# NVIDIA-Merlin/NVTabular

Hardware: NVIDIA H100
Metric: rows/sec Criteo-1TB-shaped Categorify+FillMissing+Normalize (higher is better)
Workload: dtype int64

## Files before the change

### nvtabular_b200/csrc/bucketagg.cuh

```cuda
#pragma once

namespace nvtb {

constexpr int kBkThreads = 1024;
constexpr int kBkLgParts = 13;
constexpr int kBkParts = 1 << kBkLgParts;
constexpr int kBkMaxShift = 32 - kBkLgParts;
constexpr int kBkWords = 1 << (kBkMaxShift - 5);
constexpr int kBkDupCap = 14336;
constexpr int kBkCountSmem = 4 * kBkWords;
constexpr int kBkEmitSmem = 4 * kBkWords * 2 + 2 * kBkWords + 4 * kBkDupCap;

struct PartRange {
  int lg;
  const uint32_t* par;
  __device__ __forceinline__ uint32_t xform(uint32_t k) const { return (k ^ 0x80000000u) - par[0]; }
  __device__ __forceinline__ uint32_t bin(uint32_t v) const { return v >> par[1]; }
};

static __global__ void __launch_bounds__(kPartThreads)
bk_minmax_kernel(const int32_t* __restrict__ keys, const uint8_t* __restrict__ mask, int64_t n,
                 uint32_t* __restrict__ mm, int aligned) {
  uint32_t lo = 0xFFFFFFFFu, hi = 0u;
  const int64_t n_tiles = (n + kPartTile - 1) / kPartTile;
  for (int64_t tile = blockIdx.x; tile < n_tiles; tile += gridDim.x) {
    Rows8 r[kPartGroups];
#pragma unroll
    for (int g = 0; g < kPartGroups; ++g)
      load_rows8(keys, mask, tile * kPartTile + ((int64_t)g * kPartThreads + threadIdx.x) * 8, n, r[g], aligned != 0);
#pragma unroll
    for (int g = 0; g < kPartGroups; ++g)
#pragma unroll
      for (int k = 0; k < 8; ++k)
        if ((r[g].m >> k) & 1u) {
          const uint32_t u = (uint32_t)r[g].v[k] ^ 0x80000000u;
          lo = u < lo ? u : lo;
          hi = u > hi ? u : hi;
        }
  }
#pragma unroll
  for (int o = 16; o > 0; o >>= 1) {
    const uint32_t a = __shfl_down_sync(0xFFFFFFFFu, lo, o), b = __shfl_down_sync(0xFFFFFFFFu, hi, o);
    lo = a < lo ? a : lo;
    hi = b > hi ? b : hi;
  }
  if ((threadIdx.x & 31) == 0 && lo <= hi) { atomicMin(&mm[0], lo); atomicMax(&mm[1], hi); }
}

static __global__ void bk_params_kernel(const uint32_t* __restrict__ mm, uint32_t* __restrict__ par) {
  uint32_t lo = mm[0], hi = mm[1];
  if (lo > hi) { lo = 0u; hi = 0u; }
  const uint32_t range = hi - lo;
  const int bits = range ? 32 - __clz(range) : 0;
  par[0] = lo;
  par[1] = (uint32_t)(bits > kBkLgParts ? bits - kBkLgParts : 0);
}

__device__ __forceinline__ uint32_t bk_block_sum(uint32_t v, uint32_t* ws ) {
#pragma unroll
  for (int o = 16; o > 0; o >>= 1) v += __shfl_down_sync(0xFFFFFFFFu, v, o);
  if ((threadIdx.x & 31) == 0) ws[threadIdx.x >> 5] = v;
  __syncthreads();
  uint32_t t = 0;
  if (threadIdx.x < 32) {
    t = ws[threadIdx.x];
#pragma unroll
    for (int o = 16; o > 0; o >>= 1) t += __shfl_down_sync(0xFFFFFFFFu, t, o);
    if (threadIdx.x == 0) ws[0] = t;
  }
  __syncthreads();
  t = ws[0];
  __syncthreads();
  return t;
}

__device__ __forceinline__ uint32_t bk_block_excl(uint32_t v, uint32_t* ws , uint32_t* total) {
  uint32_t incl = v;
#pragma unroll
  for (int o = 1; o < 32; o <<= 1) {
    const uint32_t y = __shfl_up_sync(0xFFFFFFFFu, incl, o);
    if ((threadIdx.x & 31) >= o) incl += y;
  }
  if ((threadIdx.x & 31) == 31) ws[threadIdx.x >> 5] = incl;
  __syncthreads();
  if (threadIdx.x < 32) {
    const uint32_t w = ws[threadIdx.x];
    uint32_t wi = w;
#pragma unroll
    for (int o = 1; o < 32; o <<= 1) {
      const uint32_t y = __shfl_up_sync(0xFFFFFFFFu, wi, o);
      if (threadIdx.x >= o) wi += y;
    }
    ws[threadIdx.x] = wi - w;
    if (threadIdx.x == 31) ws[32] = wi;
  }
  __syncthreads();
  const uint32_t ex = ws[threadIdx.x >> 5] + incl - v;
  *total = ws[32];
  __syncthreads();
  return ex;
}

static __global__ void __launch_bounds__(kBkThreads)
bk_count_kernel(const uint32_t* __restrict__ buf, const uint32_t* __restrict__ starts,
                const uint32_t* __restrict__ n_valid, const uint32_t* __restrict__ par,
                uint32_t* __restrict__ distinct) {
  extern __shared__ __align__(16) uint32_t bk_smem[];
  __shared__ uint32_t ws[33];
  uint32_t* bm = bk_smem;
  const int b = blockIdx.x;
  const uint32_t s = starts[b], e = (b + 1 < kBkParts) ? starts[b + 1] : *n_valid;
  if (s >= e) { if (threadIdx.x == 0) distinct[b] = 0u; return; }
  const uint32_t shift = par[1];
  const uint32_t wmask = (1u << shift) - 1u;
  const int words = shift > 5 ? 1 << (shift - 5) : 1;
  for (int w = threadIdx.x; w < words; w += kBkThreads) bm[w] = 0u;
  __syncthreads();
  for (uint32_t i = s + threadIdx.x; i < e; i += kBkThreads) {
    const uint32_t off = buf[i] & wmask;
    const uint32_t bit = 1u << (off & 31);
    if (!(bm[off >> 5] & bit)) atomicOr(&bm[off >> 5], bit);
  }
  __syncthreads();
  uint32_t c = 0;
  for (int w = threadIdx.x; w < words; w += kBkThreads) c += __popc(bm[w]);
  const uint32_t tot = bk_block_sum(c, ws);
  if (threadIdx.x == 0) distinct[b] = tot;
}

static __global__ void __launch_bounds__(kBkThreads)
bk_emit_kernel(const uint32_t* __restrict__ buf, const uint32_t* __restrict__ starts,
               const uint32_t* __restrict__ n_valid, const uint32_t* __restrict__ par,
               const uint32_t* __restrict__ out_base, uint64_t* __restrict__ out,
               unsigned int* __restrict__ flag, unsigned long long* __restrict__ max_count) {
  extern __shared__ __align__(16) uint32_t bk_smem[];
  __shared__ uint32_t ws[33];
  uint32_t* bm = bk_smem;
  uint32_t* dup = bm + kBkWords;
  uint16_t* pfx = reinterpret_cast<uint16_t*>(dup + kBkWords);
  uint32_t* cnt = reinterpret_cast<uint32_t*>(pfx + kBkWords);
  const int b = blockIdx.x;
  const uint32_t s = starts[b], e = (b + 1 < kBkParts) ? starts[b + 1] : *n_valid;
  if (s >= e) return;
  const uint32_t lo = par[0], shift = par[1];
  const uint32_t wmask = (1u << shift) - 1u;
  const int words = shift > 5 ? 1 << (shift - 5) : 1;
  const int per = (words + kBkThreads - 1) / kBkThreads;
  for (int w = threadIdx.x; w < words; w += kBkThreads) { bm[w] = 0u; dup[w] = 0u; }
  __syncthreads();
  for (uint32_t i = s + threadIdx.x; i < e; i += kBkThreads) {
    const uint32_t off = buf[i] & wmask;
    const uint32_t bit = 1u << (off & 31), w = off >> 5;
    const uint32_t old = atomicOr(&bm[w], bit);
    if ((old & bit) && !(dup[w] & bit)) atomicOr(&dup[w], bit);
  }
  __syncthreads();
  const int w0 = threadIdx.x * per;
  uint32_t c = 0;
  for (int j = 0; j < per; ++j) if (w0 + j < words) c += __popc(dup[w0 + j]);
  uint32_t n_dup;
  uint32_t run = bk_block_excl(c, ws, &n_dup);
  if (n_dup > (uint32_t)kBkDupCap) {
    if (threadIdx.x == 0) atomicOr(flag, 1u);
    return;
  }
  for (int j = 0; j < per; ++j)
    if (w0 + j < words) { pfx[w0 + j] = (uint16_t)run; run += __popc(dup[w0 + j]); }
  for (uint32_t i = threadIdx.x; i < n_dup; i += kBkThreads) cnt[i] = 0u;
  __syncthreads();
  if (n_dup) {
    for (uint32_t i = s + threadIdx.x; i < e; i += kBkThreads) {
      const uint32_t off = buf[i] & wmask;
      const uint32_t bit = 1u << (off & 31), w = off >> 5;
      const uint32_t d = dup[w];
      if (d & bit) atomicAdd(&cnt[pfx[w] + __popc(d & (bit - 1u))], 1u);
    }
    __syncthreads();
  }
  c = 0;
  for (int j = 0; j < per; ++j) if (w0 + j < words) c += __popc(bm[w0 + j]);
  uint32_t n_out;
  uint32_t r = bk_block_excl(c, ws, &n_out);
  uint64_t* o = out + out_base[b];
  const uint32_t vbase = lo + ((uint32_t)b << shift);
  uint32_t mx = 1u;
  for (int j = 0; j < per; ++j) {
    const int w = w0 + j;
    if (w >= words) break;
    uint32_t bits = bm[w];
    const uint32_t d = dup[w];
    const uint32_t pd = pfx[w];
    while (bits) {
      const int k = __ffs(bits) - 1;
      bits &= bits - 1u;
      uint32_t n = 1u;
      if ((d >> k) & 1u) n = cnt[pd + __popc(d & ((1u << k) - 1u))];
      mx = n > mx ? n : mx;
      o[r++] = ((uint64_t)(vbase + ((uint32_t)w << 5) + (uint32_t)k) << 32) | (uint64_t)n;
    }
  }
#pragma unroll
  for (int o2 = 16; o2 > 0; o2 >>= 1) { const uint32_t y = __shfl_down_sync(0xFFFFFFFFu, mx, o2); mx = y > mx ? y : mx; }
  if ((threadIdx.x & 31) == 0) atomicMax(max_count, (unsigned long long)mx);
}

}
```

### nvtabular_b200/csrc/sortacc.cu

```cuda
#include <algorithm>
#include <new>

#include "hashagg.cuh"
#include "partition.cuh"
#include "sortagg.cuh"
#include "bucketagg.cuh"

namespace nvtb {

struct SortedAcc {
  uint64_t* acc[2] = {nullptr, nullptr};
  int64_t acc_cap[2] = {0, 0};
  int cur = 0;
  uint32_t* d_n = nullptr;
  int32_t* stage_keys = nullptr;
  uint8_t* stage_mask = nullptr;
  int64_t stage_cap = 0;
  int64_t stage_rows = 0;
  int64_t stage_hint = 0;
  cudaEvent_t stage_ev = nullptr;
  cudaStream_t stage_last = nullptr;
};

static SharedScratch g_sort;

struct SortCarve {
  void* rx;
  size_t rx_bytes;
  uint32_t* part_meta;
  uint32_t* keys_a;
  uint32_t* keys_b;
  uint64_t* rle;
  uint32_t* tile_heads;
  uint2* splits;
  uint32_t* tile_out;
};

static size_t align_up(size_t v, size_t a) { return (v + a - 1) / a * a; }

static int sort_scratch_acquire(int64_t m, int64_t n_pairs_sort, int64_t mt, cudaStream_t st, SortCarve* c) {
  const int P = 1 << kSortLowBits;
  const size_t rx_bytes = align_up(std::max(rx_scratch_bytes<uint32_t>(m), rx_scratch_bytes<uint64_t>(n_pairs_sort)), 256);
  const size_t meta_bytes = align_up(sizeof(uint32_t) * (size_t)std::max(3 * P, 4 * kBkParts + 64), 256);
  const size_t keys_bytes = align_up(sizeof(uint32_t) * (size_t)(m + 64), 256);
  const size_t rle_bytes = align_up(sizeof(uint64_t) * (size_t)(m + 2), 256);
  const size_t heads_bytes = align_up(sizeof(uint32_t) * (size_t)((m + kRleTile - 1) / kRleTile + 1), 256);
  const size_t splits_bytes = align_up(sizeof(uint2) * (size_t)(mt + 2), 256);
  const size_t out_bytes = align_up(sizeof(uint32_t) * (size_t)(mt + 2), 256);
  const size_t need = rx_bytes + meta_bytes + 2 * keys_bytes + rle_bytes + heads_bytes + splits_bytes + out_bytes;
  void* base = nullptr;
  bool grown = false;
  int rc = g_sort.acquire(need, need + need / 8, st, &base, &grown);
  if (rc) return rc;
  if (grown) NVTB_CUDA_OK(cudaMemsetAsync(base, 0, 256, st));
  char* p = reinterpret_cast<char*>(base);
  c->rx = p;                                         p += rx_bytes;
  c->rx_bytes = rx_bytes;
  c->part_meta = reinterpret_cast<uint32_t*>(p);     p += meta_bytes;
  c->keys_a = reinterpret_cast<uint32_t*>(p);        p += keys_bytes;
  c->keys_b = reinterpret_cast<uint32_t*>(p);        p += keys_bytes;
  c->rle = reinterpret_cast<uint64_t*>(p);           p += rle_bytes;
  c->tile_heads = reinterpret_cast<uint32_t*>(p);    p += heads_bytes;
  c->splits = reinterpret_cast<uint2*>(p);           p += splits_bytes;
  c->tile_out = reinterpret_cast<uint32_t*>(p);
  return NVTB_OK;
}

static int acc_reserve(SortedAcc* a, int which, int64_t pairs, cudaStream_t st) {
  if (a->acc_cap[which] >= pairs) return NVTB_OK;
  if (a->acc[which]) NVTB_CUDA_OK(cudaFreeAsync(a->acc[which], st));
  a->acc[which] = nullptr; a->acc_cap[which] = 0;
  const int64_t want = pairs + pairs / 8 + 1024;
  NVTB_CUDA_OK(cudaMallocAsync(&a->acc[which], sizeof(uint64_t) * (size_t)want, st));
  a->acc_cap[which] = want;
  return NVTB_OK;
}

template <bool B_PACKED>
static int merge_pairs(const uint64_t* A, int64_t ua, const uint64_t* B, const uint32_t* ub_dev, int64_t mt,
                       uint64_t* out, unsigned long long* n_unique, unsigned long long* max_count, uint2* splits,
                       uint32_t* tile_out, cudaStream_t st) {
  static bool attrs = false;
  if (!attrs) {
    NVTB_CUDA_OK(cudaFuncSetAttribute(merge_write_kernel<B_PACKED>,
                                      cudaFuncAttributeMaxDynamicSharedMemorySize, (int)sizeof(MergeSmem)));
    attrs = true;
  }
  merge_split_kernel<<<(int)((mt + 1 + 255) / 256), 256, 0, st>>>(A, (uint32_t)ua, B, ub_dev, (int)mt, splits);
  NVTB_LAUNCH_OK();
  merge_count_kernel<<<(int)mt, kRunThreads, 0, st>>>(A, B, splits, tile_out);
  NVTB_LAUNCH_OK();
  scan_tiles_kernel<<<1, kRunThreads, 0, st>>>(tile_out, (int)mt, nullptr, n_unique);
  NVTB_LAUNCH_OK();
  merge_write_kernel<B_PACKED><<<(int)mt, kRunThreads, sizeof(MergeSmem), st>>>(A, B, splits, tile_out, out, max_count);
  NVTB_LAUNCH_OK();
  return NVTB_OK;
}

static int bucket_route(SortedAcc* a, const int32_t* kp, const uint8_t* mp, int64_t m, int64_t ua, Counters* ctr,
                        const SortCarve& c, cudaStream_t st, bool* ok) {
  static bool attrs = false;
  constexpr int kBkScatterSmem = kPartTile * 4 + 2 * 4 * kBkParts;
  if (!attrs) {
    NVTB_CUDA_OK(cudaFuncSetAttribute(part_hist_kernel<PartRange>, cudaFuncAttributeMaxDynamicSharedMemorySize, 4 * kBkParts));
    NVTB_CUDA_OK(cudaFuncSetAttribute(part_scatter_kernel<PartRange>, cudaFuncAttributeMaxDynamicSharedMemorySize, kBkScatterSmem));
    NVTB_CUDA_OK(cudaFuncSetAttribute(bk_count_kernel, cudaFuncAttributeMaxDynamicSharedMemorySize, kBkCountSmem));
    NVTB_CUDA_OK(cudaFuncSetAttribute(bk_emit_kernel, cudaFuncAttributeMaxDynamicSharedMemorySize, kBkEmitSmem));
    attrs = true;
  }
  const int sms = sm_count();
  const int aligned = is_aligned32(kp) ? 1 : 0;
  const int64_t tiles = (m + kPartTile - 1) / kPartTile;
  uint32_t* n_valid = a->d_n + 1;
  uint32_t* n_batch = a->d_n + 2;
  uint32_t* total = c.part_meta;
  uint32_t* cursor = c.part_meta + kBkParts;
  uint32_t* distinct = c.part_meta + 2 * kBkParts;
  uint32_t* mm = c.part_meta + 4 * kBkParts;
  uint32_t* par = mm + 2;
  unsigned int* flag = reinterpret_cast<unsigned int*>(mm + 4);
  const uint32_t mm_init[6] = {0xFFFFFFFFu, 0u, 0u, 0u, 0u, 0u};
  NVTB_CUDA_OK(cudaMemcpyAsync(mm, mm_init, sizeof(mm_init), cudaMemcpyHostToDevice, st));
  NVTB_CUDA_OK(cudaMemsetAsync(total, 0, sizeof(uint32_t) * kBkParts, st));
  bk_minmax_kernel<<<(int)std::min<int64_t>(tiles, 4 * sms), kPartThreads, 0, st>>>(kp, mp, m, mm, aligned);
  NVTB_LAUNCH_OK();
  bk_params_kernel<<<1, 1, 0, st>>>(mm, par);
  NVTB_LAUNCH_OK();
  const PartRange pol{kBkLgParts, par};
  part_hist_kernel<PartRange><<<(int)std::min<int64_t>(tiles, 3 * sms), kPartThreads, 4 * kBkParts, st>>>(
      kp, mp, m, pol, total, ctr, aligned);
  NVTB_LAUNCH_OK();
  scan_tiles_kernel<<<1, kRunThreads, 0, st>>>(total, kBkParts, n_valid, nullptr);
  NVTB_LAUNCH_OK();
  NVTB_CUDA_OK(cudaMemcpyAsync(cursor, total, sizeof(uint32_t) * kBkParts, cudaMemcpyDeviceToDevice, st));
  part_scatter_kernel<PartRange><<<(int)std::min<int64_t>(tiles, sms), kPartThreads, kBkScatterSmem, st>>>(
      kp, mp, m, pol, cursor, reinterpret_cast<int32_t*>(c.keys_a), aligned);
  NVTB_LAUNCH_OK();
  bk_count_kernel<<<kBkParts, kBkThreads, kBkCountSmem, st>>>(c.keys_a, total, n_valid, par, distinct);
  NVTB_LAUNCH_OK();
  scan_tiles_kernel<<<1, kRunThreads, 0, st>>>(distinct, kBkParts, n_batch, ua == 0 ? &ctr->n_unique : nullptr);
  NVTB_LAUNCH_OK();
  uint32_t nb_h = 0;
  NVTB_CUDA_OK(cudaMemcpyAsync(&nb_h, n_batch, sizeof(nb_h), cudaMemcpyDeviceToHost, st));
  NVTB_CUDA_OK(cudaStreamSynchronize(st));
  int rc = acc_reserve(a, a->cur ^ 1, ua + (int64_t)nb_h, st);
  if (rc) return rc;
  uint64_t* B = (ua == 0) ? a->acc[a->cur ^ 1] : c.rle;
  bk_emit_kernel<<<kBkParts, kBkThreads, kBkEmitSmem, st>>>(c.keys_a, total, n_valid, par, distinct, B, flag,
                                                             &ctr->max_count);
  NVTB_LAUNCH_OK();
  unsigned int flag_h = 0;
  NVTB_CUDA_OK(cudaMemcpyAsync(&flag_h, flag, sizeof(flag_h), cudaMemcpyDeviceToHost, st));
  NVTB_CUDA_OK(cudaStreamSynchronize(st));
  *ok = (flag_h == 0);
  return NVTB_OK;
}

static int radix_route(SortedAcc* a, const int32_t* kp, const uint8_t* mp, int64_t m, int64_t ua, Counters* null_ctr,
                       const SortCarve& c, cudaStream_t st) {
  static bool attrs = false;
  constexpr int kScatterSmem = kPartTile * 4 + 2 * 4 * (1 << kSortLowBits);
  if (!attrs) {
    NVTB_CUDA_OK(cudaFuncSetAttribute(part_scatter_kernel<PartKeyLow>,
                                      cudaFuncAttributeMaxDynamicSharedMemorySize, kScatterSmem));
    attrs = true;
  }
  const int sms = sm_count();
  const int P = 1 << kSortLowBits;
  const int aligned = is_aligned32(kp) ? 1 : 0;
  const int64_t tiles = (m + kPartTile - 1) / kPartTile;
  uint32_t* n_valid = a->d_n + 1;
  uint32_t* n_batch = a->d_n + 2;
  int rc = acc_reserve(a, a->cur ^ 1, ua + m, st);
  if (rc) return rc;
  NVTB_CUDA_OK(cudaMemsetAsync(c.part_meta, 0, sizeof(uint32_t) * P, st));
  part_hist_kernel<PartKeyLow><<<(int)std::min<int64_t>(tiles, 3 * sms), kPartThreads, 4 * P, st>>>(
      kp, mp, m, PartKeyLow{kSortLowBits}, c.part_meta, null_ctr, aligned);
  NVTB_LAUNCH_OK();
  part_scan_kernel<<<1, kPartThreads, 0, st>>>(c.part_meta, kSortLowBits, c.part_meta + P, c.part_meta + 2 * P, 1u, n_valid);
  NVTB_LAUNCH_OK();
  part_scatter_kernel<PartKeyLow><<<(int)std::min<int64_t>(tiles, 2 * sms), kPartThreads, kScatterSmem, st>>>(
      kp, mp, m, PartKeyLow{kSortLowBits}, c.part_meta + 2 * P, reinterpret_cast<int32_t*>(c.keys_a), aligned);
  NVTB_LAUNCH_OK();
  int in_b = 0;
  rc = rx_sort_bits<uint32_t>(nullptr, c.keys_a, c.keys_b, n_valid, m, kSortLowBits, 32, false, c.rx, c.rx_bytes, st,
                              &in_b);
  if (rc) return rc;
  const uint32_t* sorted = in_b ? c.keys_b : c.keys_a;
  const int rt = (int)((m + kRleTile - 1) / kRleTile);
  rle_count_kernel<<<rt, kRunThreads, 0, st>>>(sorted, n_valid, m, c.tile_heads);
  NVTB_LAUNCH_OK();
  scan_tiles_kernel<<<1, kRunThreads, 0, st>>>(c.tile_heads, rt, n_batch, nullptr);
  NVTB_LAUNCH_OK();
  rle_write_kernel<<<rt, kRunThreads, 0, st>>>(sorted, n_valid, m, c.tile_heads, n_batch, c.rle);
  NVTB_LAUNCH_OK();
  return NVTB_OK;
}

int sortacc_insert(SortedAcc* a, const int32_t* kp, const uint8_t* mp, int64_t m, int64_t ua, Counters* ctr,
                   cudaStream_t st) {
  const int64_t mt = (ua + m + kMergeTile - 1) / kMergeTile;
  SortCarve c;
  int rc = sort_scratch_acquire(m, 64, mt, st, &c);
  if (rc) return rc;
  const char* path_env = getenv("NVTB_SORT_PATH");
  const bool radix_only = path_env && strcmp(path_env, "radix") == 0;
  bool bucketed = false;
  if (!radix_only) {
    rc = bucket_route(a, kp, mp, m, ua, ctr, c, st, &bucketed);
    if (rc) return rc;
  }
  if (!bucketed) {
    rc = radix_route(a, kp, mp, m, ua, radix_only ? ctr : nullptr, c, st);
    if (rc) return rc;
  }
  const uint64_t* A = a->acc[a->cur];
  uint64_t* out = a->acc[a->cur ^ 1];
  uint32_t* n_batch = a->d_n + 2;
  if (!bucketed)
    rc = merge_pairs<false>(A, ua, c.rle, n_batch, mt, out, &ctr->n_unique, &ctr->max_count, c.splits, c.tile_out, st);
  else if (ua > 0)
    rc = merge_pairs<true>(A, ua, c.rle, n_batch, mt, out, &ctr->n_unique, &ctr->max_count, c.splits, c.tile_out, st);
  if (rc) return rc;
  a->cur ^= 1;
  return g_sort.release(st);
}

static int64_t stage_cap_rows() {
  const char* e = getenv("NVTB_STAGE_ROWS");
  int64_t v = e ? atoll(e) : ((int64_t)1 << 28);
  if (v < 0) v = 0;
  if (v > (int64_t)0xF0000000ll) v = (int64_t)0xF0000000ll;
  return v / 64 * 64;
}

int sortacc_create(SortedAcc** out, int64_t u, cudaStream_t st, uint64_t** pairs) {
  SortedAcc* a = new (std::nothrow) SortedAcc();
  NVTB_REQUIRE(a != nullptr, "host allocation failed");
  *out = a;
  *pairs = nullptr;
  NVTB_CUDA_OK(cudaMalloc(&a->d_n, sizeof(uint32_t) * 4));
  NVTB_CUDA_OK(cudaMemsetAsync(a->d_n, 0, sizeof(uint32_t) * 4, st));
  if (u > 0) {
    int rc = acc_reserve(a, 0, u, st);
    if (rc) return rc;
    rc = acc_reserve(a, 1, u, st);
    if (rc) return rc;
    *pairs = a->acc[0];
  }
  return NVTB_OK;
}

int sortacc_sort_pairs(SortedAcc* a, int64_t u, cudaStream_t st) {
  if (u == 0) return NVTB_OK;
  SortCarve c;
  int rc = sort_scratch_acquire(64, u, 1, st, &c);
  if (rc) return rc;
  int in_b = 0;
  rc = rx_sort_bits<uint64_t>(nullptr, a->acc[0], a->acc[1], nullptr, u, 32, 64, false, c.rx, c.rx_bytes, st, &in_b);
  if (rc) return rc;
  a->cur = in_b;
  return g_sort.release(st);
}

bool sortacc_stages(const SortedAcc* a, int64_t m) {
  const int64_t cap = stage_cap_rows();
  return cap >= 64 && m <= cap && (a->stage_rows & 7) == 0;
}

bool sortacc_stage_full(const SortedAcc* a, int64_t m) {
  return a->stage_rows > 0 && a->stage_rows + m > a->stage_cap;
}

int64_t sortacc_staged_rows(const SortedAcc* a) { return a->stage_rows; }

int sortacc_stage(SortedAcc* a, const int32_t* kp, const uint8_t* mp, int64_t m, int64_t rows_total, cudaStream_t st) {
  if (a->stage_ev == nullptr) NVTB_CUDA_OK(cudaEventCreateWithFlags(&a->stage_ev, cudaEventDisableTiming));
  if (a->stage_last != nullptr && a->stage_last != st) NVTB_CUDA_OK(cudaStreamWaitEvent(st, a->stage_ev, 0));
  const int64_t cap_max = stage_cap_rows();
  const bool grow_for_fit = a->stage_rows == 0 && a->stage_cap < std::min<int64_t>(cap_max, a->stage_hint);
  if (a->stage_rows + m > a->stage_cap || grow_for_fit) {
    NVTB_REQUIRE(a->stage_rows == 0, "staging buffer resized while rows are waiting");
    if (a->stage_keys) NVTB_CUDA_OK(cudaFreeAsync(a->stage_keys, st));
    if (a->stage_mask) NVTB_CUDA_OK(cudaFreeAsync(a->stage_mask, st));
    a->stage_keys = nullptr; a->stage_mask = nullptr; a->stage_cap = 0;
    int64_t want = (int64_t)1 << 22;
    while (want < 2 * (rows_total + m)) want <<= 1;
    want = std::max<int64_t>(want, (a->stage_hint + 63) / 64 * 64);
    want = std::max<int64_t>(std::min<int64_t>(want, cap_max), m);
    NVTB_CUDA_OK(cudaMallocAsync(&a->stage_keys, sizeof(int32_t) * (size_t)(want + 64), st));
    NVTB_CUDA_OK(cudaMallocAsync(&a->stage_mask, (size_t)(want / 8 + 64), st));
    a->stage_cap = want;
  }
  NVTB_CUDA_OK(cudaMemcpyAsync(a->stage_keys + a->stage_rows, kp, sizeof(int32_t) * (size_t)m, cudaMemcpyDeviceToDevice, st));
  uint8_t* md = a->stage_mask + (a->stage_rows >> 3);
  const size_t mbytes = (size_t)((m + 7) >> 3);
  if (mp) NVTB_CUDA_OK(cudaMemcpyAsync(md, mp, mbytes, cudaMemcpyDeviceToDevice, st));
  else    NVTB_CUDA_OK(cudaMemsetAsync(md, 0xFF, mbytes, st));
  a->stage_rows += m;
  NVTB_CUDA_OK(cudaEventRecord(a->stage_ev, st));
  a->stage_last = st;
  return NVTB_OK;
}

int sortacc_flush(SortedAcc* a, int64_t u, Counters* ctr, cudaStream_t st) {
  if (a->stage_rows == 0) return NVTB_OK;
  if (a->stage_last != st && a->stage_ev) NVTB_CUDA_OK(cudaStreamWaitEvent(st, a->stage_ev, 0));
  int rc = sortacc_insert(a, a->stage_keys, a->stage_mask, a->stage_rows, u, ctr, st);
  if (rc) return rc;
  a->stage_rows = 0;
  NVTB_CUDA_OK(cudaEventRecord(a->stage_ev, st));
  a->stage_last = st;
  return NVTB_OK;
}

void sortacc_reset(SortedAcc* a, int64_t rows_total) {
  a->stage_hint = std::max<int64_t>(a->stage_hint, rows_total);
  a->stage_rows = 0;
}

void sortacc_destroy(SortedAcc* a) {
  if (a->acc[0]) cudaFree(a->acc[0]);
  if (a->acc[1]) cudaFree(a->acc[1]);
  if (a->d_n) cudaFree(a->d_n);
  if (a->stage_keys) cudaFree(a->stage_keys);
  if (a->stage_mask) cudaFree(a->stage_mask);
  if (a->stage_ev) cudaEventDestroy(a->stage_ev);
  delete a;
}

const uint64_t* sortacc_pairs(const SortedAcc* a) { return a->acc[a->cur]; }

int sortacc_unpack(const SortedAcc* a, int64_t u, int64_t* keys, int64_t* sizes, cudaStream_t st) {
  runs_unpack_kernel<<<plain_grid(u), kThreads, 0, st>>>(a->acc[a->cur], u, keys, sizes);
  NVTB_LAUNCH_OK();
  return NVTB_OK;
}

}

using namespace nvtb;

extern "C" {

static int radix_sort_entry(void* data, void* tmp, int64_t n, int elem_bytes, int lo_bit, int hi_bit,
                            int descending, int* result_in_tmp_host, void* stream) {
  NVTB_REQUIRE(n >= 0 && result_in_tmp_host != nullptr, "bad n / NULL result flag");
  NVTB_REQUIRE(lo_bit >= 0 && hi_bit <= 8 * elem_bytes && lo_bit <= hi_bit, "bad bit range");
  *result_in_tmp_host = 0;
  if (n == 0 || lo_bit == hi_bit) return NVTB_OK;
  NVTB_REQUIRE(data != nullptr && tmp != nullptr, "NULL data/tmp");
  NVTB_REQUIRE((reinterpret_cast<uintptr_t>(data) & 15u) == 0 && (reinterpret_cast<uintptr_t>(tmp) & 15u) == 0,
               "data/tmp must be 16-byte aligned");
  cudaStream_t st = (cudaStream_t)stream;
  void* scratch = nullptr;
  const size_t bytes = elem_bytes == 4 ? rx_scratch_bytes<uint32_t>(n) : rx_scratch_bytes<uint64_t>(n);
  NVTB_CUDA_OK(cudaMallocAsync(&scratch, bytes, st));
  NVTB_CUDA_OK(cudaMemsetAsync(scratch, 0, 256, st));
  int rc;
  if (elem_bytes == 4)
    rc = rx_sort_bits<uint32_t>(nullptr, (uint32_t*)data, (uint32_t*)tmp, nullptr, n, lo_bit, hi_bit, descending != 0,
                                scratch, bytes, st, result_in_tmp_host);
  else
    rc = rx_sort_bits<uint64_t>(nullptr, (uint64_t*)data, (uint64_t*)tmp, nullptr, n, lo_bit, hi_bit, descending != 0,
                                scratch, bytes, st, result_in_tmp_host);
  NVTB_CUDA_OK(cudaFreeAsync(scratch, st));
  return rc;
}

int nvtb_radix_sort_u32(uint32_t* data, uint32_t* tmp, int64_t n, int lo_bit, int hi_bit, int descending,
                        int* result_in_tmp_host, void* stream) {
  return radix_sort_entry(data, tmp, n, 4, lo_bit, hi_bit, descending, result_in_tmp_host, stream);
}

int nvtb_radix_sort_u64(uint64_t* data, uint64_t* tmp, int64_t n, int lo_bit, int hi_bit, int descending,
                        int* result_in_tmp_host, void* stream) {
  return radix_sort_entry(data, tmp, n, 8, lo_bit, hi_bit, descending, result_in_tmp_host, stream);
}

int nvtb_pairs_lower_bounds(const uint64_t* pairs, int64_t n, const uint32_t* bounds_dev, int m,
                            int64_t* out_dev, void* stream) {
  NVTB_REQUIRE(n >= 0 && m >= 0, "negative size");
  if (m == 0) return NVTB_OK;
  NVTB_REQUIRE(bounds_dev != nullptr && out_dev != nullptr && (n == 0 || pairs != nullptr), "NULL argument");
  pairs_lower_bound_kernel<<<(m + 127) / 128, 128, 0, (cudaStream_t)stream>>>(
      pairs, n, bounds_dev, m, reinterpret_cast<long long*>(out_dev));
  NVTB_LAUNCH_OK();
  return NVTB_OK;
}

int nvtb_pairs_merge(const uint64_t* a, int64_t na, const uint64_t* b, int64_t nb, uint64_t* out,
                     int64_t* n_out_host, void* stream) {
  NVTB_REQUIRE(na >= 0 && nb >= 0 && n_out_host != nullptr, "bad sizes / NULL n_out");
  NVTB_REQUIRE(na + nb < (int64_t)0xFFFF0000ll, "more than 2^32 pairs in one merge");
  cudaStream_t st = (cudaStream_t)stream;
  *n_out_host = 0;
  if (na + nb == 0) return NVTB_OK;
  NVTB_REQUIRE(out != nullptr, "NULL out");
  if (na == 0 || nb == 0) {
    NVTB_CUDA_OK(cudaMemcpyAsync(out, na ? a : b, sizeof(uint64_t) * (size_t)(na + nb), cudaMemcpyDeviceToDevice, st));
    *n_out_host = na + nb;
    return NVTB_OK;
  }
  const int64_t mt = (na + nb + kMergeTile - 1) / kMergeTile;
  SortCarve c;
  int rc = sort_scratch_acquire(64, 64, mt, st, &c);
  if (rc) return rc;
  uint32_t* ub_dev = c.part_meta;
  unsigned long long* nu_dev = reinterpret_cast<unsigned long long*>(c.part_meta + 2);
  const uint32_t ub_h = (uint32_t)nb;
  NVTB_CUDA_OK(cudaMemsetAsync(ub_dev, 0, 64, st));
  NVTB_CUDA_OK(cudaMemcpyAsync(ub_dev, &ub_h, sizeof(ub_h), cudaMemcpyHostToDevice, st));
  rc = merge_pairs<true>(a, na, b, ub_dev, mt, out, nu_dev, nu_dev + 1, c.splits, c.tile_out, st);
  if (rc) return rc;
  unsigned long long nu_h = 0;
  NVTB_CUDA_OK(cudaMemcpyAsync(&nu_h, nu_dev, sizeof(nu_h), cudaMemcpyDeviceToHost, st));
  rc = g_sort.release(st);
  if (rc) return rc;
  NVTB_CUDA_OK(cudaStreamSynchronize(st));
  *n_out_host = (int64_t)nu_h;
  return NVTB_OK;
}

int nvtb_segment_copy_u64(const uint64_t* src, uint64_t* dst, const int64_t* seg_src_dev, const int64_t* seg_dst_dev,
                          int nseg, int64_t n, void* stream) {
  NVTB_REQUIRE(nseg >= 0 && n >= 0, "negative size");
  if (n == 0 || nseg == 0) return NVTB_OK;
  NVTB_REQUIRE(src && dst && seg_src_dev && seg_dst_dev, "NULL argument");
  segment_copy_kernel<<<plain_grid((n + 3) / 4), kThreads, 0, (cudaStream_t)stream>>>(
      src, dst, reinterpret_cast<const long long*>(seg_src_dev), reinterpret_cast<const long long*>(seg_dst_dev), nseg, n);
  NVTB_LAUNCH_OK();
  return NVTB_OK;
}

}
```

Before: 796.3 million.

## Two-level bucket partition, fused staging with min/max, and warp-parallel emit

Staging now runs a custom kernel that copies keys and mask and computes the key min/max in the same pass, so the flush path can skip the separate min/max kernel. The 8192-way scatter is split into a coarse 512-way scatter plus a 16-way refine kernel, which cuts shared-memory pressure in the scatter. The count and emit kernels get unrolled loads, and emit uses a dynamic shared-memory size with a duplicate cap derived from the largest bucket, allowing two blocks per SM. Emit output now uses a warp-cooperative prefix scan instead of per-thread serial runs. The extra refine pass adds a full read and write of the keys.

```diff
diff --git a/nvtabular_b200/csrc/bucketagg.cuh b/nvtabular_b200/csrc/bucketagg.cuh
--- a/nvtabular_b200/csrc/bucketagg.cuh
+++ b/nvtabular_b200/csrc/bucketagg.cuh
@@ -9,7 +9,6 @@
 constexpr int kBkWords = 1 << (kBkMaxShift - 5);
 constexpr int kBkDupCap = 14336;
 constexpr int kBkCountSmem = 4 * kBkWords;
-constexpr int kBkEmitSmem = 4 * kBkWords * 2 + 2 * kBkWords + 4 * kBkDupCap;
 
 struct PartRange {
   int lg;
@@ -17,6 +16,132 @@
   __device__ __forceinline__ uint32_t xform(uint32_t k) const { return (k ^ 0x80000000u) - par[0]; }
   __device__ __forceinline__ uint32_t bin(uint32_t v) const { return v >> par[1]; }
 };
+
+__device__ __forceinline__ void bk_fold_minmax(const Rows8& r, uint32_t& lo, uint32_t& hi) {
+#pragma unroll
+  for (int k = 0; k < 8; ++k)
+    if ((r.m >> k) & 1u) {
+      const uint32_t u = (uint32_t)r.v[k] ^ 0x80000000u;
+      lo = u < lo ? u : lo;
+      hi = u > hi ? u : hi;
+    }
+}
+
+__device__ __forceinline__ void bk_publish_minmax(uint32_t lo, uint32_t hi, uint32_t* mm) {
+#pragma unroll
+  for (int o = 16; o > 0; o >>= 1) {
+    const uint32_t a = __shfl_down_sync(0xFFFFFFFFu, lo, o), b = __shfl_down_sync(0xFFFFFFFFu, hi, o);
+    lo = a < lo ? a : lo;
+    hi = b > hi ? b : hi;
+  }
+  if ((threadIdx.x & 31) == 0 && lo <= hi) { atomicMin(&mm[0], lo); atomicMax(&mm[1], hi); }
+}
+
+constexpr int kBkLgFine = 4;
+constexpr int kBkFine = 1 << kBkLgFine;
+constexpr int kBkCoarse = kBkParts / kBkFine;
+struct PartRangeCoarse {
+  int lg;
+  const uint32_t* par;
+  __device__ __forceinline__ uint32_t xform(uint32_t k) const { return (k ^ 0x80000000u) - par[0]; }
+  __device__ __forceinline__ uint32_t bin(uint32_t v) const { return v >> (par[1] + kBkLgFine); }
+};
+
+static __global__ void bk_cursors_kernel(const uint32_t* __restrict__ starts, uint32_t* __restrict__ fine,
+                                         uint32_t* __restrict__ coarse) {
+  const int b = blockIdx.x * blockDim.x + threadIdx.x;
+  if (b >= kBkParts) return;
+  const uint32_t v = starts[b];
+  fine[b] = v;
+  if ((b & (kBkFine - 1)) == 0) coarse[b / kBkFine] = v;
+}
+
+constexpr int kBkRefineVals = 16;
+constexpr int kBkRefineTile = kPartThreads * kBkRefineVals;
+static __global__ void __launch_bounds__(kPartThreads, 2)
+bk_refine_kernel(const uint32_t* __restrict__ in, const uint32_t* __restrict__ starts,
+                 const uint32_t* __restrict__ n_valid, const uint32_t* __restrict__ par,
+                 uint32_t* __restrict__ cursor, uint32_t* __restrict__ out) {
+  __shared__ uint32_t bk_stage[kBkRefineTile];
+  __shared__ uint32_t cs[kBkCoarse + 1];
+  __shared__ uint32_t tp[kBkCoarse + 1];
+  __shared__ uint32_t cnt[kBkFine], delta[kBkFine];
+  constexpr int kVals = kBkRefineVals;
+  const uint32_t shift = par[1];
+  const int lane = threadIdx.x & 31;
+  for (int c = threadIdx.x; c <= kBkCoarse; c += kPartThreads) cs[c] = c < kBkCoarse ? starts[c * kBkFine] : *n_valid;
+  __syncthreads();
+  if (threadIdx.x < 32) {
+    constexpr int kPer = kBkCoarse / 32;
+    uint32_t t[kPer], loc = 0;
+#pragma unroll
+    for (int j = 0; j < kPer; ++j) {
+      const int c = lane * kPer + j;
+      t[j] = (cs[c + 1] - cs[c] + kBkRefineTile - 1) / kBkRefineTile;
+      loc += t[j];
+    }
+    uint32_t incl = loc;
+#pragma unroll
+    for (int o = 1; o < 32; o <<= 1) {
+      const uint32_t y = __shfl_up_sync(0xFFFFFFFFu, incl, o);
+      if (lane >= o) incl += y;
+    }
+    uint32_t run = incl - loc;
+#pragma unroll
+    for (int j = 0; j < kPer; ++j) { tp[lane * kPer + j] = run; run += t[j]; }
+    if (lane == 31) tp[kBkCoarse] = run;
+  }
+  __syncthreads();
+  const uint32_t n_tiles = tp[kBkCoarse];
+  for (uint32_t tile = blockIdx.x; tile < n_tiles; tile += gridDim.x) {
+    int c = 0;
+    for (int step = kBkCoarse / 2; step > 0; step >>= 1)
+      if (tp[c + step] <= tile) c += step;
+    const uint32_t b0 = cs[c] + (tile - tp[c]) * kBkRefineTile;
+    const uint32_t b1 = min(b0 + (uint32_t)kBkRefineTile, cs[c + 1]);
+    if (threadIdx.x < kBkFine) cnt[threadIdx.x] = 0u;
+    __syncthreads();
+    uint32_t v[kVals];
+#pragma unroll
+    for (int j = 0; j < kVals; ++j) {
+      const uint32_t i = b0 + j * kPartThreads + threadIdx.x;
+      v[j] = i < b1 ? __ldg(in + i) : 0u;
+    }
+#pragma unroll
+    for (int j = 0; j < kVals; ++j)
+      if (b0 + j * kPartThreads + threadIdx.x < b1) atomicAdd(&cnt[(v[j] >> shift) & (kBkFine - 1)], 1u);
+    __syncthreads();
+    if (threadIdx.x < 32) {
+      const uint32_t x = lane < kBkFine ? cnt[lane] : 0u;
+      uint32_t incl = x;
+#pragma unroll
+      for (int o = 1; o < 32; o <<= 1) {
+        const uint32_t y = __shfl_up_sync(0xFFFFFFFFu, incl, o);
+        if (lane >= o) incl += y;
+      }
+      const uint32_t off = incl - x;
+      if (lane < kBkFine) {
+        const uint32_t g0 = x ? atomicAdd(&cursor[c * kBkFine + lane], x) : 0u;
+        delta[lane] = g0 - off;
+        cnt[lane] = off;
+      }
+    }
+    __syncthreads();
+#pragma unroll
+    for (int j = 0; j < kVals; ++j)
+      if (b0 + j * kPartThreads + threadIdx.x < b1) {
+        const uint32_t p = atomicAdd(&cnt[(v[j] >> shift) & (kBkFine - 1)], 1u);
+        bk_stage[p] = v[j];
+      }
+    __syncthreads();
+    const uint32_t total = b1 - b0;
+    for (uint32_t j = threadIdx.x; j < total; j += kPartThreads) {
+      const uint32_t hv = bk_stage[j];
+      out[delta[(hv >> shift) & (kBkFine - 1)] + j] = hv;
+    }
+    __syncthreads();
+  }
+}
 
 static __global__ void __launch_bounds__(kPartThreads)
 bk_minmax_kernel(const int32_t* __restrict__ keys, const uint8_t* __restrict__ mask, int64_t n,
@@ -29,22 +154,36 @@
     for (int g = 0; g < kPartGroups; ++g)
       load_rows8(keys, mask, tile * kPartTile + ((int64_t)g * kPartThreads + threadIdx.x) * 8, n, r[g], aligned != 0);
 #pragma unroll
+    for (int g = 0; g < kPartGroups; ++g) bk_fold_minmax(r[g], lo, hi);
+  }
+  bk_publish_minmax(lo, hi, mm);
+}
+
+static __global__ void __launch_bounds__(kPartThreads)
+bk_stage_kernel(const int32_t* __restrict__ keys, const uint8_t* __restrict__ mask, int64_t n,
+                int32_t* __restrict__ dk, uint8_t* __restrict__ dm, uint32_t* __restrict__ mm, int aligned) {
+  uint32_t lo = 0xFFFFFFFFu, hi = 0u;
+  const int64_t n_tiles = (n + kPartTile - 1) / kPartTile;
+  for (int64_t tile = blockIdx.x; tile < n_tiles; tile += gridDim.x) {
+    Rows8 r[kPartGroups];
+#pragma unroll
     for (int g = 0; g < kPartGroups; ++g)
-#pragma unroll
-      for (int k = 0; k < 8; ++k)
-        if ((r[g].m >> k) & 1u) {
-          const uint32_t u = (uint32_t)r[g].v[k] ^ 0x80000000u;
-          lo = u < lo ? u : lo;
-          hi = u > hi ? u : hi;
-        }
-  }
-#pragma unroll
-  for (int o = 16; o > 0; o >>= 1) {
-    const uint32_t a = __shfl_down_sync(0xFFFFFFFFu, lo, o), b = __shfl_down_sync(0xFFFFFFFFu, hi, o);
-    lo = a < lo ? a : lo;
-    hi = b > hi ? b : hi;
-  }
-  if ((threadIdx.x & 31) == 0 && lo <= hi) { atomicMin(&mm[0], lo); atomicMax(&mm[1], hi); }
+      load_rows8(keys, mask, tile * kPartTile + ((int64_t)g * kPartThreads + threadIdx.x) * 8, n, r[g], aligned != 0);
+#pragma unroll
+    for (int g = 0; g < kPartGroups; ++g) {
+      const int64_t i = tile * kPartTile + ((int64_t)g * kPartThreads + threadIdx.x) * 8;
+      if (r[g].lv == 0xFFu) {
+        st_rows8<int32_t>(dk + i, r[g].v);
+      } else {
+#pragma unroll
+        for (int k = 0; k < 8; ++k)
+          if ((r[g].lv >> k) & 1u) dk[i + k] = r[g].v[k];
+      }
+      if (r[g].lv) dm[i >> 3] = (uint8_t)r[g].m;
+      bk_fold_minmax(r[g], lo, hi);
+    }
+  }
+  bk_publish_minmax(lo, hi, mm);
 }
 
 static __global__ void bk_params_kernel(const uint32_t* __restrict__ mm, uint32_t* __restrict__ par) {
@@ -101,26 +240,44 @@
   return ex;
 }
 
+constexpr int kBkUnroll = 4;
+
+template <typename F>
+__device__ __forceinline__ void bk_stream(const uint32_t* __restrict__ buf, uint32_t s, uint32_t e, F f) {
+  for (uint32_t i0 = s + threadIdx.x; i0 < e; i0 += kBkThreads * kBkUnroll) {
+    uint32_t v[kBkUnroll];
+#pragma unroll
+    for (int j = 0; j < kBkUnroll; ++j) {
+      const uint32_t i = i0 + j * kBkThreads;
+      v[j] = i < e ? __ldg(buf + i) : 0u;
+    }
+#pragma unroll
+    for (int j = 0; j < kBkUnroll; ++j)
+      if (i0 + j * kBkThreads < e) f(v[j]);
+  }
+}
+
 static __global__ void __launch_bounds__(kBkThreads)
 bk_count_kernel(const uint32_t* __restrict__ buf, const uint32_t* __restrict__ starts,
                 const uint32_t* __restrict__ n_valid, const uint32_t* __restrict__ par,
-                uint32_t* __restrict__ distinct) {
+                uint32_t* __restrict__ distinct, uint32_t* __restrict__ max_rows) {
   extern __shared__ __align__(16) uint32_t bk_smem[];
   __shared__ uint32_t ws[33];
   uint32_t* bm = bk_smem;
   const int b = blockIdx.x;
   const uint32_t s = starts[b], e = (b + 1 < kBkParts) ? starts[b + 1] : *n_valid;
   if (s >= e) { if (threadIdx.x == 0) distinct[b] = 0u; return; }
+  if (threadIdx.x == 0) atomicMax(max_rows, e - s);
   const uint32_t shift = par[1];
   const uint32_t wmask = (1u << shift) - 1u;
   const int words = shift > 5 ? 1 << (shift - 5) : 1;
   for (int w = threadIdx.x; w < words; w += kBkThreads) bm[w] = 0u;
   __syncthreads();
-  for (uint32_t i = s + threadIdx.x; i < e; i += kBkThreads) {
-    const uint32_t off = buf[i] & wmask;
+  bk_stream(buf, s, e, [&](uint32_t v) {
+    const uint32_t off = v & wmask;
     const uint32_t bit = 1u << (off & 31);
     if (!(bm[off >> 5] & bit)) atomicOr(&bm[off >> 5], bit);
-  }
+  });
   __syncthreads();
   uint32_t c = 0;
   for (int w = threadIdx.x; w < words; w += kBkThreads) c += __popc(bm[w]);
@@ -128,39 +285,45 @@
   if (threadIdx.x == 0) distinct[b] = tot;
 }
 
-static __global__ void __launch_bounds__(kBkThreads)
+__host__ __device__ constexpr int bk_emit_words(uint32_t shift) { return shift > 5 ? 1 << (shift - 5) : 1; }
+__host__ __device__ constexpr int bk_emit_smem(uint32_t shift, int cap) {
+  return 4 * (2 * bk_emit_words(shift) + (bk_emit_words(shift) + 1) / 2 + cap);
+}
+constexpr int kBkEmitSmem = bk_emit_smem(kBkMaxShift, kBkDupCap);
+
+static __global__ void __launch_bounds__(kBkThreads, 2)
 bk_emit_kernel(const uint32_t* __restrict__ buf, const uint32_t* __restrict__ starts,
                const uint32_t* __restrict__ n_valid, const uint32_t* __restrict__ par,
-               const uint32_t* __restrict__ out_base, uint64_t* __restrict__ out,
+               const uint32_t* __restrict__ out_base, uint64_t* __restrict__ out, uint32_t cap,
                unsigned int* __restrict__ flag, unsigned long long* __restrict__ max_count) {
   extern __shared__ __align__(16) uint32_t bk_smem[];
   __shared__ uint32_t ws[33];
-  uint32_t* bm = bk_smem;
-  uint32_t* dup = bm + kBkWords;
-  uint16_t* pfx = reinterpret_cast<uint16_t*>(dup + kBkWords);
-  uint32_t* cnt = reinterpret_cast<uint32_t*>(pfx + kBkWords);
   const int b = blockIdx.x;
   const uint32_t s = starts[b], e = (b + 1 < kBkParts) ? starts[b + 1] : *n_valid;
   if (s >= e) return;
   const uint32_t lo = par[0], shift = par[1];
   const uint32_t wmask = (1u << shift) - 1u;
-  const int words = shift > 5 ? 1 << (shift - 5) : 1;
+  const int words = bk_emit_words(shift);
+  uint32_t* bm = bk_smem;
+  uint32_t* dup = bm + words;
+  uint16_t* pfx = reinterpret_cast<uint16_t*>(dup + words);
+  uint32_t* cnt = dup + words + (words + 1) / 2;
   const int per = (words + kBkThreads - 1) / kBkThreads;
   for (int w = threadIdx.x; w < words; w += kBkThreads) { bm[w] = 0u; dup[w] = 0u; }
   __syncthreads();
-  for (uint32_t i = s + threadIdx.x; i < e; i += kBkThreads) {
-    const uint32_t off = buf[i] & wmask;
+  bk_stream(buf, s, e, [&](uint32_t v) {
+    const uint32_t off = v & wmask;
     const uint32_t bit = 1u << (off & 31), w = off >> 5;
     const uint32_t old = atomicOr(&bm[w], bit);
     if ((old & bit) && !(dup[w] & bit)) atomicOr(&dup[w], bit);
-  }
+  });
   __syncthreads();
   const int w0 = threadIdx.x * per;
   uint32_t c = 0;
   for (int j = 0; j < per; ++j) if (w0 + j < words) c += __popc(dup[w0 + j]);
   uint32_t n_dup;
   uint32_t run = bk_block_excl(c, ws, &n_dup);
-  if (n_dup > (uint32_t)kBkDupCap) {
+  if (n_dup > cap) {
     if (threadIdx.x == 0) atomicOr(flag, 1u);
     return;
   }
@@ -169,39 +332,54 @@
   for (uint32_t i = threadIdx.x; i < n_dup; i += kBkThreads) cnt[i] = 0u;
   __syncthreads();
   if (n_dup) {
-    for (uint32_t i = s + threadIdx.x; i < e; i += kBkThreads) {
-      const uint32_t off = buf[i] & wmask;
+    bk_stream(buf, s, e, [&](uint32_t v) {
+      const uint32_t off = v & wmask;
       const uint32_t bit = 1u << (off & 31), w = off >> 5;
       const uint32_t d = dup[w];
       if (d & bit) atomicAdd(&cnt[pfx[w] + __popc(d & (bit - 1u))], 1u);
-    }
-    __syncthreads();
-  }
+    });
+    __syncthreads();
+  }
+  const int lane = threadIdx.x & 31;
+  const int span = (words + 31) / 32;
+  const int q0 = (threadIdx.x >> 5) * span, q1 = min(q0 + span, words);
   c = 0;
-  for (int j = 0; j < per; ++j) if (w0 + j < words) c += __popc(bm[w0 + j]);
+  for (int w = q0 + lane; w < q1; w += 32) c += __popc(bm[w]);
+#pragma unroll
+  for (int o = 16; o > 0; o >>= 1) c += __shfl_xor_sync(0xFFFFFFFFu, c, o);
   uint32_t n_out;
-  uint32_t r = bk_block_excl(c, ws, &n_out);
+  uint32_t r = __shfl_sync(0xFFFFFFFFu, bk_block_excl(lane == 0 ? c : 0u, ws, &n_out), 0);
   uint64_t* o = out + out_base[b];
   const uint32_t vbase = lo + ((uint32_t)b << shift);
   uint32_t mx = 1u;
-  for (int j = 0; j < per; ++j) {
-    const int w = w0 + j;
-    if (w >= words) break;
-    uint32_t bits = bm[w];
-    const uint32_t d = dup[w];
-    const uint32_t pd = pfx[w];
-    while (bits) {
-      const int k = __ffs(bits) - 1;
-      bits &= bits - 1u;
-      uint32_t n = 1u;
-      if ((d >> k) & 1u) n = cnt[pd + __popc(d & ((1u << k) - 1u))];
-      mx = n > mx ? n : mx;
-      o[r++] = ((uint64_t)(vbase + ((uint32_t)w << 5) + (uint32_t)k) << 32) | (uint64_t)n;
+  for (int w0q = q0; w0q < q1; w0q += 32) {
+    const int w = w0q + lane;
+    uint32_t bits = w < q1 ? bm[w] : 0u;
+    const uint32_t n_bits = __popc(bits);
+    uint32_t incl = n_bits;
+#pragma unroll
+    for (int o2 = 1; o2 < 32; o2 <<= 1) {
+      const uint32_t y = __shfl_up_sync(0xFFFFFFFFu, incl, o2);
+      if (lane >= o2) incl += y;
+    }
+    uint32_t pos = r + incl - n_bits;
+    r += __shfl_sync(0xFFFFFFFFu, incl, 31);
+    if (bits) {
+      const uint32_t d = dup[w];
+      const uint32_t pd = pfx[w];
+      while (bits) {
+        const int k = __ffs(bits) - 1;
+        bits &= bits - 1u;
+        uint32_t n = 1u;
+        if ((d >> k) & 1u) n = cnt[pd + __popc(d & ((1u << k) - 1u))];
+        mx = n > mx ? n : mx;
+        o[pos++] = ((uint64_t)(vbase + ((uint32_t)w << 5) + (uint32_t)k) << 32) | (uint64_t)n;
+      }
     }
   }
 #pragma unroll
   for (int o2 = 16; o2 > 0; o2 >>= 1) { const uint32_t y = __shfl_down_sync(0xFFFFFFFFu, mx, o2); mx = y > mx ? y : mx; }
-  if ((threadIdx.x & 31) == 0) atomicMax(max_count, (unsigned long long)mx);
-}
-
-}
+  if (lane == 0) atomicMax(max_count, (unsigned long long)mx);
+}
+
+}
diff --git a/nvtabular_b200/csrc/sortacc.cu b/nvtabular_b200/csrc/sortacc.cu
--- a/nvtabular_b200/csrc/sortacc.cu
+++ b/nvtabular_b200/csrc/sortacc.cu
@@ -97,13 +97,22 @@
   return NVTB_OK;
 }
 
+constexpr int kDnWords = 8;
+
+static int minmax_reset(SortedAcc* a, cudaStream_t st) {
+  NVTB_CUDA_OK(cudaMemsetAsync(a->d_n + 4, 0xFF, sizeof(uint32_t), st));
+  NVTB_CUDA_OK(cudaMemsetAsync(a->d_n + 5, 0, sizeof(uint32_t), st));
+  return NVTB_OK;
+}
+
 static int bucket_route(SortedAcc* a, const int32_t* kp, const uint8_t* mp, int64_t m, int64_t ua, Counters* ctr,
-                        const SortCarve& c, cudaStream_t st, bool* ok) {
+                        bool have_minmax, const SortCarve& c, cudaStream_t st, bool* ok) {
   static bool attrs = false;
-  constexpr int kBkScatterSmem = kPartTile * 4 + 2 * 4 * kBkParts;
+  constexpr int kBkScatterSmem = kPartTile * 4 + 2 * 4 * kBkCoarse;
   if (!attrs) {
     NVTB_CUDA_OK(cudaFuncSetAttribute(part_hist_kernel<PartRange>, cudaFuncAttributeMaxDynamicSharedMemorySize, 4 * kBkParts));
-    NVTB_CUDA_OK(cudaFuncSetAttribute(part_scatter_kernel<PartRange>, cudaFuncAttributeMaxDynamicSharedMemorySize, kBkScatterSmem));
+    NVTB_CUDA_OK(cudaFuncSetAttribute(part_scatter_kernel<PartRangeCoarse>, cudaFuncAttributeMaxDynamicSharedMemorySize,
+                                      kBkScatterSmem));
     NVTB_CUDA_OK(cudaFuncSetAttribute(bk_count_kernel, cudaFuncAttributeMaxDynamicSharedMemorySize, kBkCountSmem));
     NVTB_CUDA_OK(cudaFuncSetAttribute(bk_emit_kernel, cudaFuncAttributeMaxDynamicSharedMemorySize, kBkEmitSmem));
     attrs = true;
@@ -116,38 +125,49 @@
   uint32_t* total = c.part_meta;
   uint32_t* cursor = c.part_meta + kBkParts;
   uint32_t* distinct = c.part_meta + 2 * kBkParts;
-  uint32_t* mm = c.part_meta + 4 * kBkParts;
-  uint32_t* par = mm + 2;
-  unsigned int* flag = reinterpret_cast<unsigned int*>(mm + 4);
-  const uint32_t mm_init[6] = {0xFFFFFFFFu, 0u, 0u, 0u, 0u, 0u};
-  NVTB_CUDA_OK(cudaMemcpyAsync(mm, mm_init, sizeof(mm_init), cudaMemcpyHostToDevice, st));
+  uint32_t* coarse = c.part_meta + 3 * kBkParts;
+  unsigned int* flag = reinterpret_cast<unsigned int*>(c.part_meta + 4 * kBkParts);
+  uint32_t* max_rows = a->d_n + 3;
+  uint32_t* mm = a->d_n + 4;
+  uint32_t* par = a->d_n + 6;
+  NVTB_CUDA_OK(cudaMemsetAsync(flag, 0, sizeof(unsigned int), st));
+  NVTB_CUDA_OK(cudaMemsetAsync(max_rows, 0, sizeof(uint32_t), st));
   NVTB_CUDA_OK(cudaMemsetAsync(total, 0, sizeof(uint32_t) * kBkParts, st));
-  bk_minmax_kernel<<<(int)std::min<int64_t>(tiles, 4 * sms), kPartThreads, 0, st>>>(kp, mp, m, mm, aligned);
-  NVTB_LAUNCH_OK();
+  if (!have_minmax) {
+    int rc = minmax_reset(a, st);
+    if (rc) return rc;
+    bk_minmax_kernel<<<(int)std::min<int64_t>(tiles, 4 * sms), kPartThreads, 0, st>>>(kp, mp, m, mm, aligned);
+    NVTB_LAUNCH_OK();
+  }
   bk_params_kernel<<<1, 1, 0, st>>>(mm, par);
   NVTB_LAUNCH_OK();
-  const PartRange pol{kBkLgParts, par};
   part_hist_kernel<PartRange><<<(int)std::min<int64_t>(tiles, 3 * sms), kPartThreads, 4 * kBkParts, st>>>(
-      kp, mp, m, pol, total, ctr, aligned);
+      kp, mp, m, PartRange{kBkLgParts, par}, total, ctr, aligned);
   NVTB_LAUNCH_OK();
   scan_tiles_kernel<<<1, kRunThreads, 0, st>>>(total, kBkParts, n_valid, nullptr);
   NVTB_LAUNCH_OK();
-  NVTB_CUDA_OK(cudaMemcpyAsync(cursor, total, sizeof(uint32_t) * kBkParts, cudaMemcpyDeviceToDevice, st));
-  part_scatter_kernel<PartRange><<<(int)std::min<int64_t>(tiles, sms), kPartThreads, kBkScatterSmem, st>>>(
-      kp, mp, m, pol, cursor, reinterpret_cast<int32_t*>(c.keys_a), aligned);
-  NVTB_LAUNCH_OK();
-  bk_count_kernel<<<kBkParts, kBkThreads, kBkCountSmem, st>>>(c.keys_a, total, n_valid, par, distinct);
+  bk_cursors_kernel<<<kBkParts / 256, 256, 0, st>>>(total, cursor, coarse);
+  NVTB_LAUNCH_OK();
+  part_scatter_kernel<PartRangeCoarse><<<(int)std::min<int64_t>(tiles, 2 * sms), kPartThreads, kBkScatterSmem, st>>>(
+      kp, mp, m, PartRangeCoarse{kBkLgParts - kBkLgFine, par}, coarse, reinterpret_cast<int32_t*>(c.keys_b), aligned);
+  NVTB_LAUNCH_OK();
+  bk_refine_kernel<<<(int)std::min<int64_t>(m / kBkRefineTile + kBkCoarse, 2 * sms), kPartThreads, 0, st>>>(
+      c.keys_b, total, n_valid, par, cursor, c.keys_a);
+  NVTB_LAUNCH_OK();
+  bk_count_kernel<<<kBkParts, kBkThreads, kBkCountSmem, st>>>(c.keys_a, total, n_valid, par, distinct, max_rows);
   NVTB_LAUNCH_OK();
   scan_tiles_kernel<<<1, kRunThreads, 0, st>>>(distinct, kBkParts, n_batch, ua == 0 ? &ctr->n_unique : nullptr);
   NVTB_LAUNCH_OK();
-  uint32_t nb_h = 0;
-  NVTB_CUDA_OK(cudaMemcpyAsync(&nb_h, n_batch, sizeof(nb_h), cudaMemcpyDeviceToHost, st));
+  uint32_t h[kDnWords - 2];
+  NVTB_CUDA_OK(cudaMemcpyAsync(h, n_batch, sizeof(h), cudaMemcpyDeviceToHost, st));
   NVTB_CUDA_OK(cudaStreamSynchronize(st));
+  const uint32_t nb_h = h[0], shift_h = h[5];
+  const int cap = (int)std::min<uint32_t>((uint32_t)kBkDupCap, h[1] / 2);
   int rc = acc_reserve(a, a->cur ^ 1, ua + (int64_t)nb_h, st);
   if (rc) return rc;
   uint64_t* B = (ua == 0) ? a->acc[a->cur ^ 1] : c.rle;
-  bk_emit_kernel<<<kBkParts, kBkThreads, kBkEmitSmem, st>>>(c.keys_a, total, n_valid, par, distinct, B, flag,
-                                                             &ctr->max_count);
+  bk_emit_kernel<<<kBkParts, kBkThreads, bk_emit_smem(shift_h, cap), st>>>(c.keys_a, total, n_valid, par, distinct,
+                                                                            B, (uint32_t)cap, flag, &ctr->max_count);
   NVTB_LAUNCH_OK();
   unsigned int flag_h = 0;
   NVTB_CUDA_OK(cudaMemcpyAsync(&flag_h, flag, sizeof(flag_h), cudaMemcpyDeviceToHost, st));
@@ -197,8 +217,8 @@
   return NVTB_OK;
 }
 
-int sortacc_insert(SortedAcc* a, const int32_t* kp, const uint8_t* mp, int64_t m, int64_t ua, Counters* ctr,
-                   cudaStream_t st) {
+static int insert_rows(SortedAcc* a, const int32_t* kp, const uint8_t* mp, int64_t m, int64_t ua, Counters* ctr,
+                       bool have_minmax, cudaStream_t st) {
   const int64_t mt = (ua + m + kMergeTile - 1) / kMergeTile;
   SortCarve c;
   int rc = sort_scratch_acquire(m, 64, mt, st, &c);
@@ -207,7 +227,7 @@
   const bool radix_only = path_env && strcmp(path_env, "radix") == 0;
   bool bucketed = false;
   if (!radix_only) {
-    rc = bucket_route(a, kp, mp, m, ua, ctr, c, st, &bucketed);
+    rc = bucket_route(a, kp, mp, m, ua, ctr, have_minmax, c, st, &bucketed);
     if (rc) return rc;
   }
   if (!bucketed) {
@@ -226,6 +246,11 @@
   return g_sort.release(st);
 }
 
+int sortacc_insert(SortedAcc* a, const int32_t* kp, const uint8_t* mp, int64_t m, int64_t ua, Counters* ctr,
+                   cudaStream_t st) {
+  return insert_rows(a, kp, mp, m, ua, ctr, false, st);
+}
+
 static int64_t stage_cap_rows() {
   const char* e = getenv("NVTB_STAGE_ROWS");
   int64_t v = e ? atoll(e) : ((int64_t)1 << 28);
@@ -239,8 +264,8 @@
   NVTB_REQUIRE(a != nullptr, "host allocation failed");
   *out = a;
   *pairs = nullptr;
-  NVTB_CUDA_OK(cudaMalloc(&a->d_n, sizeof(uint32_t) * 4));
-  NVTB_CUDA_OK(cudaMemsetAsync(a->d_n, 0, sizeof(uint32_t) * 4, st));
+  NVTB_CUDA_OK(cudaMalloc(&a->d_n, sizeof(uint32_t) * kDnWords));
+  NVTB_CUDA_OK(cudaMemsetAsync(a->d_n, 0, sizeof(uint32_t) * kDnWords, st));
   if (u > 0) {
     int rc = acc_reserve(a, 0, u, st);
     if (rc) return rc;
@@ -292,11 +317,15 @@
     NVTB_CUDA_OK(cudaMallocAsync(&a->stage_mask, (size_t)(want / 8 + 64), st));
     a->stage_cap = want;
   }
-  NVTB_CUDA_OK(cudaMemcpyAsync(a->stage_keys + a->stage_rows, kp, sizeof(int32_t) * (size_t)m, cudaMemcpyDeviceToDevice, st));
-  uint8_t* md = a->stage_mask + (a->stage_rows >> 3);
-  const size_t mbytes = (size_t)((m + 7) >> 3);
-  if (mp) NVTB_CUDA_OK(cudaMemcpyAsync(md, mp, mbytes, cudaMemcpyDeviceToDevice, st));
-  else    NVTB_CUDA_OK(cudaMemsetAsync(md, 0xFF, mbytes, st));
+  if (a->stage_rows == 0) {
+    int rc = minmax_reset(a, st);
+    if (rc) return rc;
+  }
+  const int64_t tiles = (m + kPartTile - 1) / kPartTile;
+  bk_stage_kernel<<<(int)std::min<int64_t>(tiles, 4 * sm_count()), kPartThreads, 0, st>>>(
+      kp, mp, m, a->stage_keys + a->stage_rows, a->stage_mask + (a->stage_rows >> 3), a->d_n + 4,
+      is_aligned32(kp) ? 1 : 0);
+  NVTB_LAUNCH_OK();
   a->stage_rows += m;
   NVTB_CUDA_OK(cudaEventRecord(a->stage_ev, st));
   a->stage_last = st;
@@ -306,7 +335,7 @@
 int sortacc_flush(SortedAcc* a, int64_t u, Counters* ctr, cudaStream_t st) {
   if (a->stage_rows == 0) return NVTB_OK;
   if (a->stage_last != st && a->stage_ev) NVTB_CUDA_OK(cudaStreamWaitEvent(st, a->stage_ev, 0));
-  int rc = sortacc_insert(a, a->stage_keys, a->stage_mask, a->stage_rows, u, ctr, st);
+  int rc = insert_rows(a, a->stage_keys, a->stage_mask, a->stage_rows, u, ctr, true, st);
   if (rc) return rc;
   a->stage_rows = 0;
   NVTB_CUDA_OK(cudaEventRecord(a->stage_ev, st));
```

Measured after the change: 844.7 million (median of 6 runs). 1.06x the previous value.
